# entn-at/exemplars_vc

Measured on AMD Instinct MI355X. Metric: spectral frames/sec converted (100 NMF iters, N=4096 dict), higher is better.
Workload: dtype f64

## Files before the change

### exemplars_vc_amd/csrc/evc_fused_all.hip

```cpp
#include "evc_fused_common.h"

namespace evc {

constexpr int AW = 4;
constexpr int AKT = 8;
constexpr int ATILES = AW * AKT;
constexpr int ATHREADS = 2 * AW * 64;
constexpr unsigned ALL_POLL_LIMIT = 1u << 17;
constexpr int ALL_STAGGER_PER_ITER = 11000;
constexpr int ALL_EXCH_PRIO = 3;
typedef unsigned all_u32x4 __attribute__((ext_vector_type(4)));
typedef long long all_i64x2 __attribute__((ext_vector_type(2)));

__device__ __forceinline__ bool all_polls_out(unsigned& polls, const int* coop_abort) {
    return ++polls > ALL_POLL_LIMIT ||
           ((polls & 63) == 0 && __hip_atomic_load(coop_abort, __ATOMIC_RELAXED, __HIP_MEMORY_SCOPE_AGENT) != 0);
}

constexpr long ALL_LDS_BUDGET = 160 * 1024 - 256;
__host__ __device__ constexpr int all_dict_row(int e) { return 4 * (((e >> 2) & 1) * 2 + (e >> 3)) + (e & 3); }
template <int MSTEPS, int C, bool KL>
struct AllShape {
    static constexpr int MT = MSTEPS > 4 ? 2 : 1;
    static constexpr int E = MT * 4 * 64;
    static constexpr int NE = MSTEPS * 64;
    static constexpr int RSTR = NE < 256 ? 256 : NE;
    static constexpr int STG = C > 0 ? 1 : (C == 0 ? NE : NE + ALL_MAX_MEMBERS - 1);
    static constexpr long REST = 8L * 2 * (AW * RSTR + 2 * E + (KL ? E : 1) + STG) + 3 * 4;
    static constexpr long dict_bytes(int pr) { return 8L * ATILES * 16 * pr; }
    static constexpr int PR_ALL = 4 * MSTEPS + 2;
    static constexpr int PR = KL ? 0
                              : REST + dict_bytes(PR_ALL) <= ALL_LDS_BUDGET       ? PR_ALL
                              : REST + dict_bytes(PR_ALL - 4) <= ALL_LDS_BUDGET   ? PR_ALL - 4
                                                                                  : 0;
    static constexpr bool LDS_DICT = C != 1 && PR > 0 && PR - 1 >= 4 * MSTEPS - 3;
};

#ifdef EVC_ALL_TIMING
#define EVC_STAMP(i)                                                                                             \
    do {                                                                                                         \
        if (a.dbg && tt0 == g - half && lane == 0 && w == 0)                                                     \
            a.dbg[(((long)blockIdx.x * 2 + half) * (2 * a.iters + 1) + step) * 4 + (i)] = __builtin_amdgcn_s_memtime(); \
    } while (0)
#else
#define EVC_STAMP(i)
#endif

#define EVC_ALL_LONE 0
#include "evc_fused_all_body.inc"
#undef EVC_ALL_LONE
#define EVC_ALL_LONE 1
#include "evc_fused_all_body.inc"
#undef EVC_ALL_LONE
#define EVC_ALL_LONE 2
#include "evc_fused_all_body.inc"
#undef EVC_ALL_LONE

template <int MSTEPS, int C, bool KL, int LONE = 0>
static hipError_t launch_all(FusedArgs a, int n_cus, hipStream_t s) {
    void (*kernel)(FusedArgs);
    if constexpr (LONE == 2) kernel = k_fused_quad<MSTEPS, C>;
    else if constexpr (LONE == 1) kernel = k_fused_lone<MSTEPS, C>;
    else kernel = k_fused_all<MSTEPS, C, KL>;
    int occ = 0;
    hipError_t e = hipOccupancyMaxActiveBlocksPerMultiprocessor(&occ, kernel, ATHREADS, 0);
    if (e != hipSuccess) return e;
    if (occ < 1) return hipErrorInvalidValue;
    long resident = n_cus;
    if (2 * resident > ALL_MAX_WGS) resident = ALL_MAX_WGS / 2;
    const int cr = C > 0 ? C : a.coop_c;
    if (C == 0 && (cr < 8 || cr > 64 || (cr & (cr - 1)))) return hipErrorInvalidValue;
    if (C < 0 && (cr < 2 || cr > ALL_MAX_MEMBERS)) return hipErrorInvalidValue;
    int pairs = (int)(resident / cr);
    const int want = (a.TT + 1) / 2;
    if (pairs > want) pairs = want;
    if (pairs < 1) return hipErrorInvalidValue;
    a.groups = 2 * pairs;
    a.stagger_cycles = (a.iters > 0 && a.iters <= 25 && a.TT >= 4L * a.groups && pairs >= 2) ? (long long)a.iters * ALL_STAGGER_PER_ITER : 0;
    if (C > 1 && (reinterpret_cast<uintptr_t>(a.coop_buf) & 15)) return hipErrorInvalidValue;
    if (C != 1) {
        e = hipMemsetAsync(a.coop_buf, 0xFF, sizeof(double) * 2 * (size_t)a.groups * cr * (C < 0 ? ALL_RS_STRIDE : 512), s);
        if (e != hipSuccess) return e;
    }
    if (C <= 0) {
        if (2L * a.groups * 512 > ALL_SLICE_ELEMS) return hipErrorInvalidValue;
        e = hipMemsetAsync(a.coop_buf + ALL_SLICE_OFFSET, 0xFF, sizeof(double) * 2 * (size_t)a.groups * 512, s);
        if (e != hipSuccess) return e;
    }
    hipLaunchKernelGGL(kernel, dim3((unsigned)(pairs * cr)), dim3(ATHREADS), 0, s, a);
    return hipGetLastError();
}

template <int MSTEPS, bool KL>
static hipError_t pick_c(const FusedArgs& a, int n_cus, hipStream_t s, bool lone_bin, bool quad_rows) {
    if constexpr (MSTEPS == 7 && !KL)
        if (lone_bin && a.M == 4 * MSTEPS - 3) switch (a.NT / ATILES) {
            case 2: return quad_rows ? launch_all<MSTEPS, 2, KL, 2>(a, n_cus, s) : launch_all<MSTEPS, 2, KL, 1>(a, n_cus, s);
            case 4: return quad_rows ? launch_all<MSTEPS, 4, KL, 2>(a, n_cus, s) : launch_all<MSTEPS, 4, KL, 1>(a, n_cus, s);
            case 8: return quad_rows ? launch_all<MSTEPS, 8, KL, 2>(a, n_cus, s) : launch_all<MSTEPS, 8, KL, 1>(a, n_cus, s);
            default: break;
        }
    switch (a.NT / ATILES) {
        case 1: return launch_all<MSTEPS, 1, KL>(a, n_cus, s);
        case 2: return launch_all<MSTEPS, 2, KL>(a, n_cus, s);
        case 4: return launch_all<MSTEPS, 4, KL>(a, n_cus, s);
        case 8:
            if constexpr (AllShape<MSTEPS, 8, KL>::LDS_DICT)
                if (a.M > 0 && a.M < AllShape<MSTEPS, 8, KL>::PR) return launch_all<MSTEPS, 8, KL>(a, n_cus, s);
            return launch_all<MSTEPS, 0, KL>(a, n_cus, s);
        case 16:
        case 32:
        case 64: return launch_all<MSTEPS, 0, KL>(a, n_cus, s);
        default: return launch_all<MSTEPS, -1, KL>(a, n_cus, s);
    }
}

int fused_all_members(int NT, int N, int eps_mode, int exact_div, int loss) {
    if (eps_mode == EVC_EPS_NONE || exact_div || (loss != EVC_LOSS_FROBENIUS && loss != EVC_LOSS_KL)) return 0;
    if (NT % ATILES) return 0;
    const int c = NT / ATILES;
    if (loss == EVC_LOSS_KL && c >= 2 && c < 16) return 0;
    return (c >= 1 && c <= ALL_MAX_MEMBERS) ? c : 0;
}

hipError_t fused_all_launch(int msteps, const FusedArgs& a, int n_cus, hipStream_t s, bool lone_bin, bool quad_rows) {
    if (a.NT % ATILES || !a.coop_buf || !a.coop_abort) return hipErrorInvalidValue;
    switch (msteps) {
        case 1: return a.loss == EVC_LOSS_KL ? pick_c<1, true>(a, n_cus, s, lone_bin, quad_rows) : pick_c<1, false>(a, n_cus, s, lone_bin, quad_rows);
        case 2: return a.loss == EVC_LOSS_KL ? pick_c<2, true>(a, n_cus, s, lone_bin, quad_rows) : pick_c<2, false>(a, n_cus, s, lone_bin, quad_rows);
        case 3: return a.loss == EVC_LOSS_KL ? pick_c<3, true>(a, n_cus, s, lone_bin, quad_rows) : pick_c<3, false>(a, n_cus, s, lone_bin, quad_rows);
        case 4: return a.loss == EVC_LOSS_KL ? pick_c<4, true>(a, n_cus, s, lone_bin, quad_rows) : pick_c<4, false>(a, n_cus, s, lone_bin, quad_rows);
        case 5: return a.loss == EVC_LOSS_KL ? pick_c<5, true>(a, n_cus, s, lone_bin, quad_rows) : pick_c<5, false>(a, n_cus, s, lone_bin, quad_rows);
        case 6: return a.loss == EVC_LOSS_KL ? pick_c<6, true>(a, n_cus, s, lone_bin, quad_rows) : pick_c<6, false>(a, n_cus, s, lone_bin, quad_rows);
        case 7: return a.loss == EVC_LOSS_KL ? pick_c<7, true>(a, n_cus, s, lone_bin, quad_rows) : pick_c<7, false>(a, n_cus, s, lone_bin, quad_rows);
        case 8: return a.loss == EVC_LOSS_KL ? pick_c<8, true>(a, n_cus, s, lone_bin, quad_rows) : pick_c<8, false>(a, n_cus, s, lone_bin, quad_rows);
        default: return hipErrorInvalidValue;
    }
}

}
```

### exemplars_vc_amd/csrc/evc_fused_all_body.inc

```
#if EVC_ALL_LONE
template <int MSTEPS, int C>
#if EVC_ALL_LONE == 2
__global__ __launch_bounds__(ATHREADS, 2) void k_fused_quad(FusedArgs a) {
    constexpr bool QUAD = true;
#else
__global__ __launch_bounds__(ATHREADS, 2) void k_fused_lone(FusedArgs a) {
    constexpr bool QUAD = false;
#endif
    constexpr bool KL = false, LONE = true;
    static_assert(MSTEPS > 4 && C > 1 && AllShape<MSTEPS, C, false>::LDS_DICT, "two bin tiles, the dictionary in LDS, direct exchange");
#else
template <int MSTEPS, int C, bool KL>
__global__ __launch_bounds__(ATHREADS, 2) void k_fused_all(FusedArgs a) {
    constexpr bool LONE = false, QUAD = false;
#endif
    using S = AllShape<MSTEPS, C, KL>;
    constexpr int DS = LONE ? MSTEPS - 1 : MSTEPS;
    constexpr bool HOIST = !KL && C >= 1;
    constexpr int MT = S::MT;
    constexpr int E = S::E;
    constexpr int NE = S::NE;
    constexpr int RSTR = S::RSTR;
    constexpr int MSP = (MSTEPS + 1) & ~1;
    constexpr int PR = S::PR;
    constexpr int TPD = 16 * PR;
    __shared__ __attribute__((aligned(16))) double s_red[2][AW * RSTR];
    __shared__ __attribute__((aligned(16))) double s_v[2][E];
    __shared__ __attribute__((aligned(16))) double s_x[2][E];
    __shared__ __attribute__((aligned(16))) double s_r[2][KL ? E : 1];
    __shared__ double s_stage[2][S::STG];
    __shared__ double s_dict[S::LDS_DICT ? ATILES * TPD : 1];
    __shared__ unsigned s_hb[2];
    __shared__ int s_fail;
    __shared__ __attribute__((aligned(16))) unsigned s_vok[HOIST ? 2 : 1][HOIST ? AW : 1];
    const int tid = threadIdx.x, lane = tid & 63;
    const int w8 = __builtin_amdgcn_readfirstlane(tid >> 6);
    const int half = w8 >> 2, w = w8 & 3, th = tid & (AW * 64 - 1);
    const int CR = C > 0 ? C : a.coop_c;
    const int member = blockIdx.x % CR;
    const int g = 2 * (blockIdx.x / CR) + half;
    double* const red = s_red[half];
    double* const vL = s_v[half];
    double* const xL = s_x[half];
    double* const rL = s_r[half];
    double* const stage = s_stage[half];
    unsigned hb = 0;
    const double* __restrict__ A1p = a.A1p;
    const double* __restrict__ A2p = a.A2p;
    f64x2* __restrict__ Hp = a.Hp;
    const int NT = a.NT;
    const long tile0 = (long)member * ATILES + w;
    const unsigned ul = (unsigned)lane;
    long sw = 0;

    const __amdgpu_buffer_rsrc_t r1 = __builtin_amdgcn_make_buffer_rsrc(const_cast<double*>(A1p), 0, NT * (MSP * 512), 0x00020000);
    const __amdgpu_buffer_rsrc_t r2 = __builtin_amdgcn_make_buffer_rsrc(const_cast<double*>(A2p), 0, NT * (MT * 2048), 0x00020000);
    const __amdgpu_buffer_rsrc_t rx = __builtin_amdgcn_make_buffer_rsrc(a.coop_buf, 0, C > 1 ? 2 * a.groups * (C * 4096) : 0, 0x00020000);
#ifdef EVC_ALL_NOFRAG
    bool nofrag_go = false;
#endif
    const unsigned ul16 = ul * 16u;
    constexpr int BL = 16 * ((MSTEPS - 1) >> 2) + 4 * ((MSTEPS - 1) & 3);
    const int rowA = w * AKT * TPD + all_dict_row(4 * (lane & 3) + ((lane & 15) >> 2)) * PR;
    const int rowB = w * AKT * TPD + all_dict_row(4 * (lane >> 4)) * PR;
    const double* const dA = s_dict + rowA + (lane >> 4);
    const double* const dAL = s_dict + rowA + min(lane >> 4, a.M - BL);
    const double* const dB = s_dict + rowB + (lane & 15);
    const double* const dBL = s_dict + rowB + min(lane & 15, a.M - 16 * (MT - 1));
    const double* const dL = s_dict + rowB + BL;
    constexpr int MTL = QUAD ? MT - 1 : MT;
    constexpr int NQ = QUAD ? MSTEPS - 4 * MTL : 0;
    const double* const dQ = s_dict + rowB + 16 * MTL + (lane & 3);
    const double* const dQL = s_dict + rowB + min(BL + (lane & 3), a.M);
#define LDS_NO_PAIR() asm volatile("" ::: "memory")
    auto load_a1 = [&](double (&a1)[DS], int k, auto lds) {
        if constexpr (decltype(lds)::value) {
#pragma unroll
            for (int s = 0; s < DS; ++s) {
                a1[s] = (s == MSTEPS - 1 ? dAL : dA)[k * TPD + 16 * (s >> 2) + 4 * (s & 3)];
                LDS_NO_PAIR();
            }
            return;
        }
        if constexpr (!LONE) {
#ifdef EVC_ALL_NOFRAG
        if (nofrag_go) return;
#endif
        const int so = (int)(tile0 + sw + AW * k) * (MSP * 512);
#pragma unroll
        for (int s = 0; s < MSTEPS; s += 2) {
            if (s + 1 < MSTEPS) {
                const f64x2 v = __builtin_bit_cast(f64x2, __builtin_amdgcn_raw_buffer_load_b128(r1, ul16 + (s >> 1) * 1024, so, 0));
                a1[s] = v[0];
                a1[s + 1] = v[1];
            } else {
                a1[s] = __builtin_bit_cast(double, __builtin_amdgcn_raw_buffer_load_b64(r1, ul16 + (s >> 1) * 1024, so, 0));
            }
        }
        }
    };
    auto load_lone = [&](double (&al)[4], int k) {
#pragma unroll
        for (int r = 0; r < 4; ++r) {
            al[r] = dL[k * TPD + r * PR];
            LDS_NO_PAIR();
        }
    };
    auto load_a2 = [&](double (&a2)[MT][4], int k, auto lds) {
        if constexpr (decltype(lds)::value) {
#pragma unroll
            for (int u = 0; u < MTL; ++u)
#pragma unroll
                for (int r = 0; r < 4; ++r) {
                    a2[u][r] = (u == MT - 1 ? dBL : dB)[k * TPD + r * PR + 16 * u];
                    LDS_NO_PAIR();
                }
            return;
        }
#ifdef EVC_ALL_NOFRAG
        if (nofrag_go) return;
#endif
        const int so = (int)(tile0 + sw + AW * k) * (MT * 2048);
#pragma unroll
        for (int u = 0; u < MT; ++u)
#pragma unroll
            for (int r = 0; r < 4; r += 2) {
                const f64x2 v = __builtin_bit_cast(f64x2, __builtin_amdgcn_raw_buffer_load_b128(r2, ul16 + (u * 2 + (r >> 1)) * 1024, so, 0));
                a2[u][r] = v[0];
                a2[u][r + 1] = v[1];
            }
    };
    auto load_aq = [&](double (&aq)[NQ > 0 ? NQ : 1][4], int k) {
#pragma unroll
        for (int r = 0; r < 4; ++r)
#pragma unroll
            for (int b = 0; b < NQ; ++b) {
                aq[b][r] = b < NQ - 1 ? dQ[k * TPD + r * PR + 4 * b] : dQL[k * TPD + r * PR];
                LDS_NO_PAIR();
            }
    };

    const int mode = a.eps_mode;
    const double eps = a.eps;
    const double d0 = a.l1 + (mode == EVC_EPS_ADD ? a.eps : 0.0);
    const f64x4 dinit = {d0, d0, d0, d0};
    const unsigned lo = fast_lo(mode, eps);
    unsigned seq = 0;
    bool tame = false;
    int rs_es = 1, rs_len = 0, rs_pub0 = 0, rs_pub1 = 0, rs_src0 = -1, rs_src1 = -1, rs_src2 = -1;
    if (C < 0) {
        rs_es = (NE + CR - 1) / CR;
        rs_len = NE - member * rs_es;
        rs_len = rs_len < 0 ? 0 : (rs_len > rs_es ? rs_es : rs_len);
        const int e0 = th, e1 = th + AW * 64;
        const int j0 = e0 / rs_es, j1 = (e1 < NE ? e1 : e0) / rs_es;
        rs_pub0 = (j0 * CR + member) * rs_es + (e0 - j0 * rs_es);
        rs_pub1 = (j1 * CR + member) * rs_es + ((e1 < NE ? e1 : e0) - j1 * rs_es);
        auto src = [&](int idx) {
            if (idx >= CR * rs_es) return -1;
            const int el = idx % rs_es;
            return el < rs_len ? member * CR * rs_es + idx : -1;
        };
        rs_src0 = src(th);
        rs_src1 = src(th + AW * 64);
        rs_src2 = src(th + 2 * AW * 64);
    }
    if (tid == 0) s_fail = 0;
    if (tid < 2) s_hb[tid] = 0;

    if (a.stagger_cycles > 0 && ((blockIdx.x / CR) & 1)) {
        const long long t0 = __builtin_amdgcn_s_memtime();
        while (__builtin_amdgcn_s_memtime() - t0 < a.stagger_cycles) __builtin_amdgcn_s_sleep(32);
    }

    auto run = [&](auto lds) __attribute__((always_inline)) {
    for (long tt0 = g - half; tt0 < a.TT; tt0 += a.groups) {
        const long tt = tt0 + half;
        bool valid;
        {
            const long t = 16 * tt + (lane & 15);
            int u = -1;
            if (tt < a.TT && t < a.T_) u = a.frame_utt[t];
            const bool live = tt < a.TT && ((t >= a.T_) || ((u >= 0) && (a.active[u] != 0)));
            const int v0 = __syncthreads_and(half == 0 ? live : true);
            const int v1 = __syncthreads_and(half == 1 ? live : true);
            valid = (half ? v1 : v0) != 0;
        }
        HTile h[AKT];
        f64x4 p[AKT];
        double a1[DS], a2[MT][4], al[4];
        if (valid && a.first && a.init_const) {
            auto h0_of = [&](int fr) {
                const long t = 16 * tt + fr;
                const int u = t < a.T_ ? a.frame_utt[t] : -1;
                return u >= 0 ? a.h0[u] : 0.0;
            };
            for (int e = th; e < E; e += AW * 64) {
                const int s = e >> 6, l = e & 63;
                const bool in = s < MSTEPS;
                xL[e] = in ? a.Xp[(tt * MSTEPS + s) * 64 + l] : 0.0;
                vL[e] = in ? a.rsum[bin_of(s, l >> 4)] * h0_of(l & 15) : 0.0;
                if (KL) rL[e] = xL[e] / (vL[e] < a.eps ? a.eps : vL[e]);
            }
            const double hv = h0_of(lane & 15);
#pragma unroll
            for (int k = 0; k < AKT; ++k) {
                const long n0 = 16 * (tile0 + AW * k) + 4 * (lane >> 4);
#pragma unroll
                for (int r = 0; r < 4; ++r) h[k][r] = n0 + r < a.N ? hv : 0.0;
            }
        } else if (valid) {
            for (int e = th; e < E; e += AW * 64) {
                const int s = e >> 6, l = e & 63;
                const bool in = s < MSTEPS;
                xL[e] = in ? a.Xp[(tt * MSTEPS + s) * 64 + l] : 0.0;
                vL[e] = in ? a.Vp[(tt * 8 + s) * 64 + l] : 0.0;
                if (KL) rL[e] = xL[e] / (vL[e] < a.eps ? a.eps : vL[e]);
            }
#pragma unroll
            for (int k = 0; k < AKT; ++k) {
                const f64x2* t = Hp + (tt * NT + tile0 + AW * k) * 128;
                const f64x2 h01 = t[ul], h23 = t[ul + 64];
                h[k][0] = h01[0]; h[k][1] = h01[1]; h[k][2] = h23[0]; h[k][3] = h23[1];
            }
        }
        if constexpr (HOIST) {
            if (lane == 0) s_vok[half][w] = 0u;
        }
        __syncthreads();
        if (valid && !KL) {
            double x[DS], xl = 0.0;
#pragma unroll
            for (int s = 0; s < DS; ++s) x[s] = xL[s * 64 + lane];
            if constexpr (LONE) xl = xL[DS * 64 + (lane & 15)];
            load_a1(a1, 0, lds);
            if constexpr (LONE) load_lone(al, 0);
#pragma unroll
            for (int k = 0; k < AKT; ++k) {
                f64x4 acc = {0, 0, 0, 0};
                if constexpr (LONE) {
#pragma unroll
                    for (int r = 0; r < 4; ++r) acc[r] = al[r] * xl;
                }
#pragma unroll
                for (int s = 0; s < DS; ++s) acc = Mma<double>::mma(a1[s], x[s], acc);
                if (!decltype(lds)::value || k + 1 < AKT) load_a1(a1, (k + 1) % AKT, lds);
                if constexpr (LONE) {
                    if (k + 1 < AKT) load_lone(al, k + 1);
                }
                p[k] = acc;
            }
        }

        if (valid && KL) load_a1(a1, 0, lds);
        for (int step = 0; step <= 2 * a.iters; ++step) {
#ifdef EVC_ALL_NOFRAG
            nofrag_go = step > 2;
#endif
            const bool mine = C == 1 ? (step & 1) == 0 : (step & 1) == half;
            EVC_STAMP(0);
            if (valid && mine && step < 2 * a.iters) {
                asm volatile("" : "+s"(sw));
                double v[DS], vl = 0.0;
#pragma unroll
                for (int s = 0; s < DS; ++s) {
                    v[s] = KL ? rL[s * 64 + lane] : vL[s * 64 + lane];
                    if constexpr (HOIST && MSTEPS == 2 && decltype(lds)::value) LDS_NO_PAIR();
                }
                if constexpr (LONE) vl = vL[DS * 64 + (lane & 15)];
                bool safe = false;
                if constexpr (HOIST) {
                    static_assert(AW == 4, "the half's four words are one 16-byte read");
                    const all_u32x4 ok4 = *reinterpret_cast<const all_u32x4*>(s_vok[half]);
                    safe = tame && __builtin_amdgcn_readfirstlane((int)(ok4[0] & ok4[1] & ok4[2] & ok4[3])) != 0;
                }
                if constexpr (decltype(lds)::value) load_a1(a1, 0, lds);
                f64x4 dl = dinit;
                if constexpr (LONE) {
                    load_lone(al, 0);
#pragma unroll
                    for (int r = 0; r < 4; ++r) dl[r] = __builtin_fma(al[r], vl, d0);
                }
                EVC_STAMP(3);
                f64x4 vn[MT];
#pragma unroll
                for (int u = 0; u < MT; ++u) vn[u] = f64x4{0, 0, 0, 0};
                double vq[NQ > 0 ? NQ : 1] = {};
#pragma unroll
                for (int k = 0; k < AKT; ++k) {
                    __builtin_amdgcn_sched_barrier(0);
                    load_a2(a2, k, lds);
                    f64x4 d = KL ? f64x4{0, 0, 0, 0} : (LONE ? dl : dinit);
#pragma unroll
                    for (int s = 0; s < DS; ++s) d = Mma<double>::mma(a1[s], v[s], d);
                    if (!decltype(lds)::value || k + 1 < AKT)
                        load_a1(a1, (k + 1) % AKT, lds);
                    if constexpr (LONE) {
                        if (k + 1 < AKT) load_lone(al, k + 1);
                    }
                    __builtin_amdgcn_sched_barrier(0);
                    if constexpr (LONE) {
                        if (k + 1 < AKT) {
                            asm volatile("" : "+v"(al[0]), "+v"(al[1]), "+v"(al[2]), "+v"(al[3]));
#pragma unroll
                            for (int r = 0; r < 4; ++r) dl[r] = __builtin_fma(al[r], vl, d0);
                        }
                    }
                    if (KL) {
#pragma unroll
                        for (int r = 0; r < 4; ++r) h[k][r] *= d[r];
                    } else if constexpr (HOIST) {
                        mu_tile_hoisted(h[k], p[k], d, mode, eps, lo, safe);
                    } else {
                        mu_tile_guarded(h[k], p[k], d, mode, eps, lo);
                    }
                    if constexpr (C >= 1) __builtin_amdgcn_sched_barrier(0);
                    [[maybe_unused]] double aq[NQ > 0 ? NQ : 1][4];
                    if constexpr (QUAD) load_aq(aq, k);
#pragma unroll
                    for (int u = 0; u < MTL; ++u)
#pragma unroll
                        for (int r = 0; r < 4; ++r) vn[u] = Mma<double>::mma(a2[u][r], h[k][r], vn[u]);
                    if constexpr (QUAD) {
#pragma unroll
                        for (int r = 0; r < 4; ++r)
#pragma unroll
                            for (int b = 0; b < NQ; ++b)
                                vq[b] = __builtin_amdgcn_mfma_f64_4x4x4f64(aq[b][r], h[k][r], vq[b], 0, 0, 0);
                    }
                }
#pragma unroll
                for (int u = 0; u < MTL; ++u)
#pragma unroll
                    for (int r = 0; r < 4; ++r)
                        if (u * 4 + r < MSTEPS) red[w * RSTR + (u * 4 + r) * 64 + lane] = vn[u][r];
                if constexpr (QUAD) {
#pragma unroll
                    for (int b = 0; b < NQ; ++b) red[w * RSTR + (4 * MTL + b) * 64 + lane] = vq[b];
                }
            } else if (C > 1 && valid && !mine && step > 0) {
                __builtin_amdgcn_s_setprio(ALL_EXCH_PRIO);
                const bool act = th < NE / 2;
                const int ep = act ? 2 * th : 0;
                f64x2 sm = {0.0, 0.0};
                unsigned vok = 1u;
                if (w * 64 < NE / 2) {
                    f64x2 pv[AW];
#pragma unroll
                    for (int ww = 0; ww < AW; ++ww) pv[ww] = *reinterpret_cast<const f64x2*>(red + ww * RSTR + ep);
                    static_assert(AW == 4, "the four partials are named one by one");
                    asm volatile("" : "+v"(pv[0]), "+v"(pv[1]), "+v"(pv[2]), "+v"(pv[3]));
#pragma unroll
                    for (int ww = 0; ww < AW; ++ww) sm += pv[ww];
                    const long long tag = (seq >> 1) & 1;
                    const long long m0 = (__double_as_longlong(sm[0]) & ~1LL) | tag;
                    const long long m1 = (__double_as_longlong(sm[1]) & ~1LL) | tag;
                    const int xo = __builtin_amdgcn_readfirstlane((int)(((seq & 1) * (unsigned)a.groups + (unsigned)g) * (unsigned)(C * 4096)));
                    if (act)
                        __builtin_amdgcn_raw_buffer_store_b128(__builtin_bit_cast(all_u32x4, all_i64x2{m0, m1}), rx, ep * 8,
                                                               xo + member * 4096, 16);
                    bool ok = true;
                    unsigned polls = 0;
                    {
                        const long long* sp = reinterpret_cast<const long long*>(a.coop_buf) +
                                              ((size_t)(seq & 1) * a.groups + g) * (size_t)(C * 512) +
                                              (lane < C ? lane : 0) * 512 + (NE - 1);
                        for (;;) {
                            const long long b = __hip_atomic_load(sp, __ATOMIC_RELAXED, __HIP_MEMORY_SCOPE_AGENT);
                            const bool ready = lane >= C || lane == member || (b & 1) == tag;
                            if (__all(ready)) break;
                            if (all_polls_out(polls, a.coop_abort)) {
                                ok = false;
                                break;
                            }
                            __builtin_amdgcn_s_sleep(2);
                        }
                    }
                    all_i64x2 b[C > 0 ? C : 1] = {};
                    polls = 0;
                    while (__builtin_expect(ok && act, 1)) {
                        asm volatile("" ::: "memory");
#pragma unroll
                        for (int m = 0; m < C; ++m)
                            if (m != member)
                                b[m] = __builtin_bit_cast(all_i64x2, __builtin_amdgcn_raw_buffer_load_b128(rx, ep * 8, xo + m * 4096, 16));
                        long long bad = 0;
#pragma unroll
                        for (int m = 0; m < C; ++m) {
                            b[m] = (m == member) ? all_i64x2{m0, m1} : b[m];
                            bad |= (b[m][0] ^ tag) | (b[m][1] ^ tag);
                        }
                        if ((bad & 1) == 0) break;
                        if (all_polls_out(polls, a.coop_abort)) {
                            ok = false;
                            break;
                        }
                        __builtin_amdgcn_s_sleep(2);
                    }
                    f64x2 v2 = {0.0, 0.0};
#pragma unroll
                    for (int m = 0; m < C; ++m) {
                        v2[0] += __longlong_as_double(b[m][0] & ~1LL);
                        v2[1] += __longlong_as_double(b[m][1] & ~1LL);
                    }
                    if (!ok) s_fail = 1;
                    if constexpr (HOIST) {
                        const bool real = act && bin_of(ep >> 6, (ep & 63) >> 4) < a.M;
                        vok = __all(!real || (range_v_ok(v2[0]) && range_v_ok(v2[1]))) ? 1u : 0u;
                    }
                    if (act) {
                        *reinterpret_cast<f64x2*>(vL + ep) = v2;
                        if (KL) {
                            const f64x2 x2 = *reinterpret_cast<const f64x2*>(xL + ep);
                            *reinterpret_cast<f64x2*>(rL + ep) =
                                f64x2{x2[0] / (v2[0] < a.eps ? a.eps : v2[0]), x2[1] / (v2[1] < a.eps ? a.eps : v2[1])};
                        }
                    }
                }
                if constexpr (HOIST) {
                    if (lane == 0) s_vok[half][w] = vok;
                }
                ++seq;
                __builtin_amdgcn_s_setprio(0);
            } else if (valid && !mine && step > 0) {
                const int e0 = C <= 0 ? th % NE : th, e1 = th + AW * 64;
                const bool has1 = e1 < NE;
                __builtin_amdgcn_s_setprio(ALL_EXCH_PRIO);
                double s0 = 0.0, s1 = 0.0;
#pragma unroll
                for (int ww = 0; ww < AW; ++ww) {
                    s0 += red[ww * RSTR + e0];
                    s1 += red[ww * RSTR + (has1 ? e1 : e0)];
                }
                if (C < 0) {
                    long long* xb1 = reinterpret_cast<long long*>(a.coop_buf) +
                                     ((size_t)(seq & 1) * a.groups + g) * (size_t)CR * ALL_RS_STRIDE;
                    long long* xb2 = reinterpret_cast<long long*>(a.coop_buf) + ALL_SLICE_OFFSET +
                                     ((size_t)(seq & 1) * a.groups + g) * 512;
                    const long long tag = (seq >> 1) & 1;
                    __hip_atomic_store(xb1 + rs_pub0, (__double_as_longlong(s0) & ~1LL) | tag, __ATOMIC_RELAXED,
                                       __HIP_MEMORY_SCOPE_AGENT);
                    if (has1)
                        __hip_atomic_store(xb1 + rs_pub1, (__double_as_longlong(s1) & ~1LL) | tag, __ATOMIC_RELAXED,
                                           __HIP_MEMORY_SCOPE_AGENT);
                    bool ok = true;
                    auto fetch3 = [&](const long long* p0, const long long* p1, const long long* p2, long long& b0,
                                      long long& b1, long long& b2) {
                        unsigned polls = 0;
                        for (;;) {
                            b0 = __hip_atomic_load(p0, __ATOMIC_RELAXED, __HIP_MEMORY_SCOPE_AGENT);
                            b1 = __hip_atomic_load(p1, __ATOMIC_RELAXED, __HIP_MEMORY_SCOPE_AGENT);
                            b2 = __hip_atomic_load(p2, __ATOMIC_RELAXED, __HIP_MEMORY_SCOPE_AGENT);
                            if (__all(!ok || (((b0 ^ tag) | (b1 ^ tag) | (b2 ^ tag)) & 1) == 0)) break;
                            if (all_polls_out(polls, a.coop_abort))
                                ok = false;
                            __builtin_amdgcn_s_sleep(1);
                        }
                    };
                    {
                        long long b0, b1, b2;
                        const long long* own = xb1 + rs_pub0;
                        fetch3(rs_src0 >= 0 ? xb1 + rs_src0 : own, rs_src1 >= 0 ? xb1 + rs_src1 : own,
                               rs_src2 >= 0 ? xb1 + rs_src2 : own, b0, b1, b2);
                        if (rs_src0 >= 0) stage[th] = __longlong_as_double(b0 & ~1LL);
                        if (rs_src1 >= 0) stage[th + AW * 64] = __longlong_as_double(b1 & ~1LL);
                        if (rs_src2 >= 0) stage[th + 2 * AW * 64] = __longlong_as_double(b2 & ~1LL);
                        hb += AW;
                        if (lane == 0)
                            __hip_atomic_fetch_add(&s_hb[half], 1u, __ATOMIC_RELEASE, __HIP_MEMORY_SCOPE_WORKGROUP);
                        while ((int)(__hip_atomic_load(&s_hb[half], __ATOMIC_ACQUIRE, __HIP_MEMORY_SCOPE_WORKGROUP) - hb) < 0)
                            __builtin_amdgcn_s_sleep(1);
                        const int q = th & 3;
                        for (int el = th >> 2; el < rs_len; el += AW * 16) {
                            double v = 0.0;
                            for (int m = q; m < CR; m += 4) v += stage[m * rs_es + el];
                            v += __shfl_xor(v, 1, 64);
                            v += __shfl_xor(v, 2, 64);
                            if (q == 0)
                                __hip_atomic_store(xb2 + member * rs_es + el, (__double_as_longlong(v) & ~1LL) | tag,
                                                   __ATOMIC_RELAXED, __HIP_MEMORY_SCOPE_AGENT);
                        }
                    }
                    long long g0, g1, g2;
                    fetch3(xb2 + e0, xb2 + (has1 ? e1 : e0), xb2 + e0, g0, g1, g2);
                    s0 = __longlong_as_double(g0 & ~1LL);
                    s1 = __longlong_as_double(g1 & ~1LL);
                    ++seq;
                    if (!ok) s_fail = 1;
                } else if (C == 0) {
                    const int ES = NE / CR;
                    long long* xb1 = reinterpret_cast<long long*>(a.coop_buf) +
                                     ((size_t)(seq & 1) * a.groups + g) * (size_t)CR * 512;
                    long long* xb2 = reinterpret_cast<long long*>(a.coop_buf) + ALL_SLICE_OFFSET +
                                     ((size_t)(seq & 1) * a.groups + g) * 512;
                    const long long tag = (seq >> 1) & 1;
                    {
                        const int j0 = e0 / ES, j1 = (has1 ? e1 : e0) / ES;
                        __hip_atomic_store(xb1 + ((size_t)j0 * CR + member) * ES + (e0 - j0 * ES),
                                           (__double_as_longlong(s0) & ~1LL) | tag, __ATOMIC_RELAXED,
                                           __HIP_MEMORY_SCOPE_AGENT);
                        if (has1)
                            __hip_atomic_store(xb1 + ((size_t)j1 * CR + member) * ES + (e1 - j1 * ES),
                                               (__double_as_longlong(s1) & ~1LL) | tag, __ATOMIC_RELAXED,
                                               __HIP_MEMORY_SCOPE_AGENT);
                    }
                    bool ok = true;
                    auto fetch2 = [&](const long long* p0, const long long* p1, long long& b0, long long& b1) {
                        unsigned polls = 0;
                        for (;;) {
                            b0 = __hip_atomic_load(p0, __ATOMIC_RELAXED, __HIP_MEMORY_SCOPE_AGENT);
                            b1 = __hip_atomic_load(p1, __ATOMIC_RELAXED, __HIP_MEMORY_SCOPE_AGENT);
                            if (__all(!ok || (((b0 ^ tag) | (b1 ^ tag)) & 1) == 0)) break;
                            if (all_polls_out(polls, a.coop_abort))
                                ok = false;
                            __builtin_amdgcn_s_sleep(1);
                        }
                    };
                    {
                        long long b0, b1;
                        const long long* mine_ = xb1 + (size_t)member * NE;
                        fetch2(mine_ + e0, mine_ + (has1 ? e1 : e0), b0, b1);
                        stage[e0] = __longlong_as_double(b0 & ~1LL);
                        if (has1) stage[e1] = __longlong_as_double(b1 & ~1LL);
                        hb += AW;
                        if (lane == 0)
                            __hip_atomic_fetch_add(&s_hb[half], 1u, __ATOMIC_RELEASE, __HIP_MEMORY_SCOPE_WORKGROUP);
                        while ((int)(__hip_atomic_load(&s_hb[half], __ATOMIC_ACQUIRE, __HIP_MEMORY_SCOPE_WORKGROUP) - hb) < 0)
                            __builtin_amdgcn_s_sleep(1);
                        if (th < 4 * ES) {
                            const int el = th >> 2, q = th & 3, per = CR >> 2;
                            double v = 0.0;
                            for (int i = 0; i < per; ++i) v += stage[(q * per + i) * ES + el];
                            v += __shfl_xor(v, 1, 64);
                            v += __shfl_xor(v, 2, 64);
                            if (q == 0)
                                __hip_atomic_store(xb2 + member * ES + el, (__double_as_longlong(v) & ~1LL) | tag,
                                                   __ATOMIC_RELAXED, __HIP_MEMORY_SCOPE_AGENT);
                        }
                    }
                    long long g0, g1;
                    fetch2(xb2 + e0, xb2 + (has1 ? e1 : e0), g0, g1);
                    s0 = __longlong_as_double(g0 & ~1LL);
                    s1 = __longlong_as_double(g1 & ~1LL);
                    ++seq;
                    if (!ok) s_fail = 1;
                }
                vL[e0] = s0;
                if (has1) vL[e1] = s1;
                if constexpr (HOIST) {
                    const bool real0 = e0 < NE && bin_of(e0 >> 6, (e0 & 63) >> 4) < a.M;
                    const bool real1 = has1 && bin_of(e1 >> 6, (e1 & 63) >> 4) < a.M;
                    const unsigned vok = __all((!real0 || range_v_ok(s0)) && (!real1 || range_v_ok(s1))) ? 1u : 0u;
                    if (lane == 0) s_vok[half][w] = vok;
                }
                if (KL) {
                    rL[e0] = xL[e0] / (s0 < a.eps ? a.eps : s0);
                    if (has1) rL[e1] = xL[e1] / (s1 < a.eps ? a.eps : s1);
                }
                __builtin_amdgcn_s_setprio(0);
            }
            EVC_STAMP(1);
            __syncthreads();
            EVC_STAMP(2);
            if (C != 1 && s_fail) {
                if (tid == 0) __hip_atomic_store(a.coop_abort, 1, __ATOMIC_RELAXED, __HIP_MEMORY_SCOPE_AGENT);
                return;
            }
        }

        auto y_tail = [&](auto ut) __attribute__((always_inline)) {
            constexpr int UT = decltype(ut)::value;
            f64x4 yn[UT];
#pragma unroll
            for (int u = 0; u < UT; ++u) yn[u] = f64x4{0, 0, 0, 0};
            if (valid) {
                const __amdgpu_buffer_rsrc_t rb = __builtin_amdgcn_make_buffer_rsrc(const_cast<double*>(a.Yb2p), 0, NT * (UT * 2048), 0x00020000);
#pragma unroll
                for (int k = 0; k < AKT; ++k) {
                    const int so = (int)(tile0 + AW * k) * (UT * 2048);
                    double b2[UT][4];
#pragma unroll
                    for (int u = 0; u < UT; ++u)
#pragma unroll
                        for (int r = 0; r < 4; r += 2) {
                            const f64x2 v = __builtin_bit_cast(f64x2, __builtin_amdgcn_raw_buffer_load_b128(rb, ul16 + (u * 2 + (r >> 1)) * 1024, so, 0));
                            b2[u][r] = v[0];
                            b2[u][r + 1] = v[1];
                        }
#pragma unroll
                    for (int u = 0; u < UT; ++u)
#pragma unroll
                        for (int r = 0; r < 4; ++r) yn[u] = Mma<double>::mma(b2[u][r], h[k][r], yn[u]);
                }
            }
#pragma unroll
            for (int u = 0; u < UT; ++u) {
                if (valid) {
#pragma unroll
                    for (int r = 0; r < 4; ++r) red[w * RSTR + r * 64 + lane] = yn[u][r];
                }
                __syncthreads();
                if (valid) {
                    double y = 0.0;
#pragma unroll
                    for (int ww = 0; ww < AW; ++ww) y += red[ww * RSTR + th];
                    a.Yslab[member * a.y_stride + (tt * 8 + 4 * u) * 64 + th] = y;
                }
                __syncthreads();
            }
        };
        if (a.Yslab) {
            if (MT > 1 && a.y_mt == 1) y_tail(std::integral_constant<int, 1>{});
            else y_tail(std::integral_constant<int, MT>{});
        }
        if (valid) {
            if (!a.skip_hp) {
#pragma unroll
                for (int k = 0; k < AKT; ++k) {
                    f64x2* t = Hp + (tt * NT + tile0 + AW * k) * 128;
                    t[ul] = f64x2{h[k][0], h[k][1]};
                    t[ul + 64] = f64x2{h[k][2], h[k][3]};
                }
            }
            if (a.Hx) {
                const long t = 16 * tt + (lane & 15);
                if (t < a.T_ && a.hx_wide) {
#pragma unroll
                    for (int k = 0; k < AKT; ++k) {
                        const long n0 = 16 * (tile0 + AW * k) + 4 * (lane >> 4);
                        double* const row = a.Hx + t * a.ldhx + n0;
#pragma unroll
                        for (int r = 0; r < 4; r += 2) {
                            if (n0 + r + 1 < a.N) *reinterpret_cast<f64x2*>(row + r) = f64x2{h[k][r], h[k][r + 1]};
                            else if (n0 + r < a.N) row[r] = h[k][r];
                        }
                    }
                } else if (t < a.T_) {
#pragma unroll
                    for (int k = 0; k < AKT; ++k) {
                        const long n0 = 16 * (tile0 + AW * k) + 4 * (lane >> 4);
#pragma unroll
                        for (int r = 0; r < 4; ++r)
                            if (n0 + r < a.N) {
                                if (a.hx_frame_major) a.Hx[t * a.ldhx + n0 + r] = h[k][r];
                                else a.Hx[(n0 + r) * a.ldhx + t] = h[k][r];
                            }
                    }
                }
            }
            if (member == 0) {
                for (int e = th; e < NE; e += AW * 64) a.Vp[(tt * 8 + (e >> 6)) * 64 + (e & 63)] = vL[e];
                if (a.write_err && w == 0) {
                    double e = 0.0;
#pragma unroll
                    for (int s = 0; s < MSTEPS; ++s) {
                        const double x = xL[s * 64 + lane], vv = vL[s * 64 + lane];
                        e += KL ? kl_terms(x, vv, a.eps) : (x - vv) * (x - vv);
                    }
                    e += __shfl_xor(e, 16, 64);
                    e += __shfl_xor(e, 32, 64);
                    const long t = 16 * tt + lane;
                    if (lane < 16 && t < a.T_) a.err2[t] = e;
                }
            }
        }
        __syncthreads();
    }
    };

    if constexpr (HOIST) {
        static_assert(ATHREADS == 16 * ATILES, "one thread per exemplar of the member");
        const long j = (long)member * ATILES + (tid >> 4);
        const int e = tid & 15, q = e >> 2, r = e & 3;
        bool ok = a.range_hoist != 0 && a.M > 0 && a.M <= 16 * MT && 16 * j + e < a.N && d0 >= 0.0 && d0 <= RANGE_SUM_HI &&
                  lo <= RANGE_LO_MAX;
        if (ok) {
            double cs = 0.0;
            for (int b = 0; b < a.M; ++b) {
                const double x = A2p[((j * MT + (b >> 4)) * 2 + (r >> 1)) * 128 + (16 * q + (b & 15)) * 2 + (r & 1)];
                ok = ok && x >= 0.0;
                cs += x;
            }
            ok = ok && cs >= RANGE_SUM_LO && cs <= RANGE_SUM_HI;
        }
        tame = __builtin_amdgcn_readfirstlane(__syncthreads_and(ok)) != 0;
    }
    if constexpr (S::LDS_DICT) {
        if (LONE ? a.M == 4 * MSTEPS - 3 : (a.M > 0 && a.M < PR)) {
            for (int x = tid; x < ATILES * TPD; x += ATHREADS) {
                const int slot = x / TPD, e = all_dict_row((x / PR) % 16), b = x % PR;
                const long j = (long)member * ATILES + slot / AKT + AW * (slot % AKT);
                const int q = e >> 2, r = e & 3;
                s_dict[x] = b < a.M ? A2p[((j * MT + (b >> 4)) * 2 + (r >> 1)) * 128 + (16 * q + (b & 15)) * 2 + (r & 1)] : 0.0;
            }
            __syncthreads();
            run(std::true_type{});
            return;
        }
    }
    if constexpr (!LONE) run(std::false_type{});
}
```

Measured before the change: 1.261 million.

## Add specialized quad-row cross-WG exchange with last-element ballot polling

```diff
diff --git a/exemplars_vc_amd/csrc/evc_fused_all.hip b/exemplars_vc_amd/csrc/evc_fused_all.hip
--- a/exemplars_vc_amd/csrc/evc_fused_all.hip
+++ b/exemplars_vc_amd/csrc/evc_fused_all.hip
@@ -9,6 +9,7 @@
 constexpr unsigned ALL_POLL_LIMIT = 1u << 17;
 constexpr int ALL_STAGGER_PER_ITER = 11000;
 constexpr int ALL_EXCH_PRIO = 3;
+typedef unsigned all_u32x2 __attribute__((ext_vector_type(2)));
 typedef unsigned all_u32x4 __attribute__((ext_vector_type(4)));
 typedef long long all_i64x2 __attribute__((ext_vector_type(2)));
 
diff --git a/exemplars_vc_amd/csrc/evc_fused_all_body.inc b/exemplars_vc_amd/csrc/evc_fused_all_body.inc
--- a/exemplars_vc_amd/csrc/evc_fused_all_body.inc
+++ b/exemplars_vc_amd/csrc/evc_fused_all_body.inc
@@ -165,6 +165,12 @@
         rs_src1 = src(th + AW * 64);
         rs_src2 = src(th + 2 * AW * 64);
     }
+    unsigned long long xq_peers = 0, xq_real = 0;
+    if constexpr (QUAD) {
+        xq_peers = __builtin_amdgcn_ballot_w64(lane < C && lane != member);
+        xq_real = __builtin_amdgcn_ballot_w64(th < NE / 2 && bin_of((2 * th) >> 6, ((2 * th) & 63) >> 4) < a.M);
+        asm volatile("" : "+s"(xq_peers), "+s"(xq_real));
+    }
     if (tid == 0) s_fail = 0;
     if (tid < 2) s_hb[tid] = 0;
 
@@ -338,6 +344,80 @@
 #pragma unroll
                     for (int b = 0; b < NQ; ++b) red[w * RSTR + (4 * MTL + b) * 64 + lane] = vq[b];
                 }
+            } else if (QUAD && valid && !mine && step > 0) {
+                constexpr int CQ = C > 0 ? C : 1;
+                __builtin_amdgcn_s_setprio(ALL_EXCH_PRIO);
+                const bool act = th < NE / 2;
+                const int ep = act ? 2 * th : 0;
+                unsigned vok = 1u;
+                if (w * 64 < NE / 2) {
+                    f64x2 pv[AW], sm = {0.0, 0.0};
+#pragma unroll
+                    for (int ww = 0; ww < AW; ++ww) pv[ww] = *reinterpret_cast<const f64x2*>(red + ww * RSTR + ep);
+                    static_assert(AW == 4, "the four partials are named one by one");
+                    asm volatile("" : "+v"(pv[0]), "+v"(pv[1]), "+v"(pv[2]), "+v"(pv[3]));
+#pragma unroll
+                    for (int ww = 0; ww < AW; ++ww) sm += pv[ww];
+                    unsigned tag = (seq >> 1) & 1;
+                    all_u32x4 pw = __builtin_bit_cast(all_u32x4, sm);
+                    pw[0] = (pw[0] & ~1u) | tag;
+                    pw[2] = (pw[2] & ~1u) | tag;
+                    const int xo = __builtin_amdgcn_readfirstlane((int)(((seq & 1) * (unsigned)a.groups + (unsigned)g) * (unsigned)(C * 4096)));
+                    if (act) __builtin_amdgcn_raw_buffer_store_b128(pw, rx, ep * 8, xo + member * 4096, 16);
+                    bool ok = true;
+                    unsigned polls = 0;
+                    const int wo = (lane < C ? lane : 0) * 4096 + (NE - 1) * 8;
+                    for (;;) {
+                        asm volatile("" ::: "memory");
+                        all_u32x2 b = __builtin_amdgcn_raw_buffer_load_b64(rx, wo, xo, 16);
+                        asm volatile("" : "+v"(b));
+                        if ((__builtin_amdgcn_ballot_w64(((b[0] ^ tag) & 1) != 0) & xq_peers) == 0) break;
+                        if (all_polls_out(polls, a.coop_abort)) {
+                            ok = false;
+                            break;
+                        }
+                        __builtin_amdgcn_s_sleep(2);
+                    }
+                    all_i64x2 b[CQ];
+#pragma unroll
+                    for (int m = 0; m < CQ; ++m) asm volatile("" : "=v"(b[m]));
+                    unsigned rounds = 0;
+                    while (__builtin_expect(ok && act, 1)) {
+                        asm volatile("" ::: "memory");
+#pragma unroll
+                        for (int m = 0; m < CQ; ++m)
+                            b[m] = __builtin_bit_cast(all_i64x2, __builtin_amdgcn_raw_buffer_load_b128(rx, ep * 8, xo + m * 4096, 16));
+                        unsigned stale = 0;
+                        if (tag) {
+#pragma unroll
+                            for (int m = 0; m < CQ; ++m) stale |= ~(unsigned)b[m][0] | ~(unsigned)b[m][1];
+                        } else {
+#pragma unroll
+                            for (int m = 0; m < CQ; ++m) stale |= (unsigned)b[m][0] | (unsigned)b[m][1];
+                        }
+                        if ((stale & 1) == 0) break;
+                        unsigned r = __builtin_amdgcn_readfirstlane(rounds);
+                        const bool out = all_polls_out(r, a.coop_abort);
+                        rounds = r;
+                        if (out) {
+                            ok = false;
+                            break;
+                        }
+                        __builtin_amdgcn_s_sleep(2);
+                    }
+                    f64x2 v2 = {0.0, 0.0};
+#pragma unroll
+                    for (int m = 0; m < CQ; ++m) {
+                        v2[0] += __longlong_as_double(b[m][0] & ~1LL);
+                        v2[1] += __longlong_as_double(b[m][1] & ~1LL);
+                    }
+                    if (!ok) s_fail = 1;
+                    vok = (__builtin_amdgcn_ballot_w64(!(range_v_ok(v2[0]) && range_v_ok(v2[1]))) & xq_real) == 0 ? 1u : 0u;
+                    if (act) *reinterpret_cast<f64x2*>(vL + ep) = v2;
+                }
+                if (lane == 0) s_vok[half][w] = vok;
+                ++seq;
+                __builtin_amdgcn_s_setprio(0);
             } else if (C > 1 && valid && !mine && step > 0) {
                 __builtin_amdgcn_s_setprio(ALL_EXCH_PRIO);
                 const bool act = th < NE / 2;
```

Result: faster. 1.285 million (median of 6 runs) (+1.9%).
